# PJLab-ADG/OpenPCSeg

Measured on AMD Instinct MI355X. Metric: LiDAR frames/sec training MinkUNet-34 SemanticKITTI, higher is better.
Workload: dtype f32; 1 GPU; MinkUNet-34 cr1.0 train step, 12 x 120k-pt synthetic SemanticKITTI scans/GPU, fp32; global_batch=12, voxels_per_gpu_batch=1158864, parallelism=dp1, wgrad=fp32

## Files before the change

### openpcseg_amd/csrc/conv_wgrad.hip

```cpp
#include "conv_common.h"

using namespace pcs;

namespace {

constexpr int WG_PB = 32;
constexpr int WG_TS = 128 + 16;

struct WgradArgs {
  const float *fa;
  const float *fb;
  const int32_t *pairs;
  const int32_t *koff;
  float *partial;
  int ca, cb, K, a_col, pch;
};

__device__ __forceinline__ void find_split(const int32_t *koff, int K, int pch, int split, int *k_out,
                                           int *beg, int *end) {
  int acc = 0;
  for (int k = 0; k < K; ++k) {
    const int nk = koff[k + 1] - koff[k];
    const int ns = (nk + pch - 1) / pch;
    if (split < acc + ns) {
      const int s = split - acc;
      *k_out = k;
      *beg = koff[k] + s * pch;
      const int e = *beg + pch;
      *end = e < koff[k + 1] ? e : koff[k + 1];
      return;
    }
    acc += ns;
  }
  *k_out = -1; *beg = 0; *end = 0;
}

__device__ __forceinline__ void find_split_wave(const int32_t *koff, int K, int pch, int split, int lane, int *beg,
                                                int *end, int *gsid, int interleave) {
  if (K > 64) {
    int k;
    find_split(koff, K, pch, split, &k, beg, end);
    *gsid = split;
    return;
  }
  const int lo = lane < K ? koff[lane] : 0, hi = lane < K ? koff[lane + 1] : 0;
  const int ns = (hi - lo + pch - 1) / pch;
  int incl = ns;
  for (int o = 1; o < 64; o <<= 1) {
    const int t = __shfl_up(incl, o, 64);
    if (lane >= o) incl += t;
  }
  int src, sidx;
  if (!interleave) {
    const unsigned long long hit = __ballot(split >= incl - ns && split < incl);
    if (!hit) { *beg = 0; *end = 0; *gsid = split; return; }
    src = __ffsll((long long)hit) - 1;
    sidx = split - __shfl(incl - ns, src, 64);
  } else {
    const int total = __shfl(incl, 63, 64);
    if (interleave == 2) {
      const int chunk = (total + 7) >> 3;
      split = (split & 7) * chunk + (split >> 3);
    }
    if (split >= total) { *beg = 0; *end = 0; *gsid = 0; return; }
    int rmax = ns;
    for (int o = 32; o > 0; o >>= 1) { const int t = __shfl_xor(rmax, o, 64); rmax = t > rmax ? t : rmax; }
    auto upto = [&](int r) {
      int c = ns > 0 ? (int)(((long long)r * ns) / rmax) + 1 : 0;
      for (int o = 32; o > 0; o >>= 1) c += __shfl_xor(c, o, 64);
      return c;
    };
    int a = 0, b = rmax - 1;
    while (a < b) {
      const int m = (a + b) >> 1;
      if (upto(m) > split) b = m; else a = m + 1;
    }
    const int r = a;
    const int before = r > 0 ? upto(r - 1) : 0;
    const int s_r = ns > 0 ? (int)(((long long)r * ns) / rmax) : -1;
    const int s_p = (ns > 0 && r > 0) ? (int)(((long long)(r - 1) * ns) / rmax) : -1;
    unsigned long long fresh = __ballot(ns > 0 && s_r != s_p);
    int want = split - before;
    while (want > 0) { fresh &= fresh - 1; --want; }
    src = __ffsll((long long)fresh) - 1;
    sidx = __shfl(s_r, src, 64);
  }
  const int b0 = lo + sidx * pch;
  const int e0 = b0 + pch < hi ? b0 + pch : hi;
  *beg = __shfl(b0, src, 64);
  *end = __shfl(e0, src, 64);
  *gsid = __shfl(incl - ns, src, 64) + sidx;
}

template <bool VEC>
__global__ void __launch_bounds__(256) wgrad_kernel(WgradArgs w) {
  __shared__ __attribute__((aligned(16))) float abuf[WG_PB * WG_TS];
  __shared__ __attribute__((aligned(16))) float bbuf[WG_PB * WG_TS];
  __shared__ int ia[WG_PB], ib[WG_PB];
  __shared__ int sh[3];
  const int tid = threadIdx.x, lane = tid & 63, wid = tid >> 6;
  const int a0 = blockIdx.y * 128, b0 = blockIdx.z * 128;
  const int cat = (w.ca - a0) < 128 ? (w.ca - a0) : 128;
  const int cbt = (w.cb - b0) < 128 ? (w.cb - b0) : 128;
  const int ta_n = (cat + 15) / 16, tb_n = (cbt + 15) / 16;
  if (tid == 0) find_split(w.koff, w.K, w.pch, blockIdx.x, &sh[0], &sh[1], &sh[2]);
  __syncthreads();
  const int beg = sh[1], end = sh[2];
  const int wa = wid >> 1, wb = wid & 1;
  f32x4 acc[4][4];
#pragma unroll
  for (int i = 0; i < 4; ++i)
#pragma unroll
    for (int j = 0; j < 4; ++j) acc[i][j] = (f32x4){0, 0, 0, 0};

  const int capad = ta_n * 16, cbpad = tb_n * 16;
  for (int p0 = beg; p0 < end; p0 += WG_PB) {
    const int np = (end - p0) < WG_PB ? (end - p0) : WG_PB;
    __syncthreads();
    if (tid < WG_PB) {
      int2 p = make_int2(-1, -1);
      if (tid < np) p = reinterpret_cast<const int2 *>(w.pairs)[p0 + tid];
      ia[tid] = w.a_col ? p.y : p.x;
      ib[tid] = w.a_col ? p.x : p.y;
    }
    __syncthreads();
    if (VEC) {
      for (int e = tid; e < WG_PB * (capad / 4); e += 256) {
        const int r = e / (capad / 4), c4 = (e % (capad / 4)) * 4;
        float4 v = make_float4(0.f, 0.f, 0.f, 0.f);
        if (r < np && c4 < cat) v = *reinterpret_cast<const float4 *>(w.fa + (int64_t)ia[r] * w.ca + a0 + c4);
        *reinterpret_cast<float4 *>(abuf + r * WG_TS + c4) = v;
      }
      for (int e = tid; e < WG_PB * (cbpad / 4); e += 256) {
        const int r = e / (cbpad / 4), c4 = (e % (cbpad / 4)) * 4;
        float4 v = make_float4(0.f, 0.f, 0.f, 0.f);
        if (r < np && c4 < cbt) v = *reinterpret_cast<const float4 *>(w.fb + (int64_t)ib[r] * w.cb + b0 + c4);
        *reinterpret_cast<float4 *>(bbuf + r * WG_TS + c4) = v;
      }
    } else {
      for (int e = tid; e < WG_PB * capad; e += 256) {
        const int r = e / capad, c = e % capad;
        abuf[r * WG_TS + c] = (r < np && c < cat) ? w.fa[(int64_t)ia[r] * w.ca + a0 + c] : 0.f;
      }
      for (int e = tid; e < WG_PB * cbpad; e += 256) {
        const int r = e / cbpad, c = e % cbpad;
        bbuf[r * WG_TS + c] = (r < np && c < cbt) ? w.fb[(int64_t)ib[r] * w.cb + b0 + c] : 0.f;
      }
    }
    __syncthreads();
    const int g = lane >> 4, l15 = lane & 15;
#pragma unroll
    for (int kk = 0; kk < WG_PB / 4; ++kk) {
      float av[4], bv[4];
#pragma unroll
      for (int i = 0; i < 4; ++i) {
        const int ta = wa + 2 * i;
        av[i] = (ta < ta_n) ? abuf[(kk * 4 + g) * WG_TS + ta * 16 + l15] : 0.f;
      }
#pragma unroll
      for (int j = 0; j < 4; ++j) {
        const int tb = wb + 2 * j;
        bv[j] = (tb < tb_n) ? bbuf[(kk * 4 + g) * WG_TS + tb * 16 + l15] : 0.f;
      }
#pragma unroll
      for (int i = 0; i < 4; ++i) {
        if (wa + 2 * i < ta_n) {
#pragma unroll
          for (int j = 0; j < 4; ++j) {
            if (wb + 2 * j < tb_n)
              acc[i][j] = __builtin_amdgcn_mfma_f32_16x16x4f32(av[i], bv[j], acc[i][j], 0, 0, 0);
          }
        }
      }
    }
  }
  float *out = w.partial + (int64_t)blockIdx.x * w.ca * w.cb;
  const int g = lane >> 4, l15 = lane & 15;
#pragma unroll
  for (int i = 0; i < 4; ++i) {
    const int ta = wa + 2 * i;
    if (ta >= ta_n) continue;
#pragma unroll
    for (int j = 0; j < 4; ++j) {
      const int tb = wb + 2 * j;
      if (tb >= tb_n) continue;
#pragma unroll
      for (int r = 0; r < 4; ++r) {
        const int ra = ta * 16 + g * 4 + r, cbv = tb * 16 + l15;
        if (ra < cat && cbv < cbt) out[(int64_t)(a0 + ra) * w.cb + b0 + cbv] = acc[i][j][r];
      }
    }
  }
}

__global__ void __launch_bounds__(256) wgrad_reduce_kernel(const float *__restrict__ partial,
                                                           const int32_t *__restrict__ koff,
                                                           int K, int pch, int64_t cc,
                                                           float *__restrict__ gW) {
  const int k = blockIdx.y;
  __shared__ int sh[2];
  if (threadIdx.x == 0) {
    int acc = 0;
    for (int q = 0; q < k; ++q) acc += (koff[q + 1] - koff[q] + pch - 1) / pch;
    sh[0] = acc;
    sh[1] = (koff[k + 1] - koff[k] + pch - 1) / pch;
  }
  __syncthreads();
  const int base = sh[0], ns = sh[1];
  for (int64_t e = (int64_t)blockIdx.x * blockDim.x + threadIdx.x; e < cc;
       e += (int64_t)gridDim.x * blockDim.x) {
    float s = 0.f;
    for (int q = 0; q < ns; ++q) s += partial[(int64_t)(base + q) * cc + e];
    gW[(int64_t)k * cc + e] = s;
  }
}

__global__ void __launch_bounds__(256) wgrad_reduce4_kernel(const float *__restrict__ partial,
                                                            const int32_t *__restrict__ koff,
                                                            int K, int pch, int64_t cc,
                                                            float *__restrict__ gW) {
  const int k = blockIdx.y;
  __shared__ int sh[2];
  __shared__ float4 red[16][16];
  if (threadIdx.x < 64) {
    const int lane = threadIdx.x;
    int acc = 0, mine = 0;
    if (K <= 64) {
      const int nsq = lane < K ? (koff[lane + 1] - koff[lane] + pch - 1) / pch : 0;
      int incl = nsq;
      for (int o = 1; o < 64; o <<= 1) {
        const int t = __shfl_up(incl, o, 64);
        if (lane >= o) incl += t;
      }
      acc = __shfl(incl - nsq, k, 64);
      mine = __shfl(nsq, k, 64);
    } else {
      for (int q = 0; q < k; ++q) acc += (koff[q + 1] - koff[q] + pch - 1) / pch;
      mine = (koff[k + 1] - koff[k] + pch - 1) / pch;
    }
    if (lane == 0) { sh[0] = acc; sh[1] = mine; }
  }
  __syncthreads();
  const int base = sh[0], ns = sh[1];
  const int et = threadIdx.x & 15, ql = threadIdx.x >> 4;
  const int64_t e = ((int64_t)blockIdx.x * 16 + et) * 4;
  const bool ok = e < cc;
  const float *p = partial + (int64_t)base * cc + (ok ? e : 0);
  float4 s0 = {0, 0, 0, 0}, s1 = s0, s2 = s0, s3 = s0;
  int q = ql;
  for (; q + 48 < ns; q += 64) {
    const float4 v0 = *reinterpret_cast<const float4 *>(p + (int64_t)q * cc);
    const float4 v1 = *reinterpret_cast<const float4 *>(p + (int64_t)(q + 16) * cc);
    const float4 v2 = *reinterpret_cast<const float4 *>(p + (int64_t)(q + 32) * cc);
    const float4 v3 = *reinterpret_cast<const float4 *>(p + (int64_t)(q + 48) * cc);
    s0.x += v0.x; s0.y += v0.y; s0.z += v0.z; s0.w += v0.w;
    s1.x += v1.x; s1.y += v1.y; s1.z += v1.z; s1.w += v1.w;
    s2.x += v2.x; s2.y += v2.y; s2.z += v2.z; s2.w += v2.w;
    s3.x += v3.x; s3.y += v3.y; s3.z += v3.z; s3.w += v3.w;
  }
  for (; q < ns; q += 16) {
    const float4 v0 = *reinterpret_cast<const float4 *>(p + (int64_t)q * cc);
    s0.x += v0.x; s0.y += v0.y; s0.z += v0.z; s0.w += v0.w;
  }
  s0.x += s1.x + (s2.x + s3.x); s0.y += s1.y + (s2.y + s3.y);
  s0.z += s1.z + (s2.z + s3.z); s0.w += s1.w + (s2.w + s3.w);
  red[ql][et] = s0;
  __syncthreads();
  if (ql == 0 && ok) {
    float4 t = red[0][et];
#pragma unroll
    for (int j = 1; j < 16; ++j) {
      const float4 v = red[j][et];
      t.x += v.x; t.y += v.y; t.z += v.z; t.w += v.w;
    }
    *reinterpret_cast<float4 *>(gW + (int64_t)k * cc + e) = t;
  }
}

struct Wgrad2Args {
  const void *fa;
  const void *fb;
  const int32_t *pairs;
  const int32_t *koff;
  float *partial;
  int ca, cb, K, a_col, pch, nbg;
  int interleave;
};

__host__ __device__ inline int wg_ngroups(int c) { return (c + 63) / 64; }
__host__ __device__ inline int wg_gwidth(int c) {
  const int per = (c + wg_ngroups(c) - 1) / wg_ngroups(c);
  return (per + 15) / 16 * 16;
}

template <int W> struct WVec;
template <> struct WVec<64> { using T = float4; static constexpr int N = 4; };
template <> struct WVec<48> { using T = float3; static constexpr int N = 3; };
template <> struct WVec<32> { using T = float2; static constexpr int N = 2; };
template <> struct WVec<16> { using T = float;  static constexpr int N = 1; };
__device__ __forceinline__ float wcomp(const float4 &v, int i) { return i == 0 ? v.x : (i == 1 ? v.y : (i == 2 ? v.z : v.w)); }
__device__ __forceinline__ float wcomp(const float3 &v, int i) { return i == 0 ? v.x : (i == 1 ? v.y : v.z); }
__device__ __forceinline__ float wcomp(const float2 &v, int i) { return i == 0 ? v.x : v.y; }
__device__ __forceinline__ float wcomp(const float &v, int) { return v; }

template <typename V, int N> __device__ __forceinline__ V wload(Fp32, const void *base, int64_t elem) {
  return *reinterpret_cast<const V *>(reinterpret_cast<const float *>(base) + elem);
}
template <typename V, int N, typename HT> __device__ __forceinline__ V wload(HT, const void *base, int64_t elem) {
  const uint16_t *p = reinterpret_cast<const uint16_t *>(base) + elem;
  V v;
  if constexpr (N == 4) {
    const uint2 r = *reinterpret_cast<const uint2 *>(p);
    v.x = h2f(HT{}, (uint16_t)(r.x & 0xFFFFu)); v.y = h2f(HT{}, (uint16_t)(r.x >> 16));
    v.z = h2f(HT{}, (uint16_t)(r.y & 0xFFFFu)); v.w = h2f(HT{}, (uint16_t)(r.y >> 16));
  } else if constexpr (N == 3) {
    v.x = h2f(HT{}, p[0]); v.y = h2f(HT{}, p[1]); v.z = h2f(HT{}, p[2]);
  } else if constexpr (N == 2) {
    const uint32_t r = *reinterpret_cast<const uint32_t *>(p);
    v.x = h2f(HT{}, (uint16_t)(r & 0xFFFFu)); v.y = h2f(HT{}, (uint16_t)(r >> 16));
  } else {
    v = h2f(HT{}, p[0]);
  }
  return v;
}

template <int AW, int BW, typename ET>
__device__ __forceinline__ void wgrad_block(const Wgrad2Args &w, int a0, int b0, int beg, int end,
                                            float *out, int lane) {
  using AV = typename WVec<AW>::T;
  using BV = typename WVec<BW>::T;
  constexpr int NA = WVec<AW>::N, NB = WVec<BW>::N;
  const int g = lane >> 4, l15 = lane & 15;
  const int ac = a0 + NA * l15, bc = b0 + NB * l15;
  const bool aok = ac + NA <= w.ca, bok = bc + NB <= w.cb;
  const int acl = aok ? ac : 0, bcl = bok ? bc : 0;
  f32x4 acc[NA][NB];
#pragma unroll
  for (int f = 0; f < NA; ++f)
#pragma unroll
    for (int h = 0; h < NB; ++h) acc[f][h] = (f32x4){0, 0, 0, 0};

  struct Batch { AV a[4]; BV b[4]; };
  auto load_pairs = [&](int p0) {
    int pi = p0 + l15;
    pi = pi < end ? pi : end - 1;
    return reinterpret_cast<const int2 *>(w.pairs)[pi];
  };
  auto load_rows = [&](Batch &bt, const int2 pr) {
    const int ia = w.a_col ? pr.y : pr.x, ib = w.a_col ? pr.x : pr.y;
#pragma unroll
    for (int j = 0; j < 4; ++j) {
      const int ra = __shfl(ia, 4 * j + g, 64), rb = __shfl(ib, 4 * j + g, 64);
      bt.a[j] = wload<AV, NA>(ET{}, w.fa, (int64_t)ra * w.ca + acl);
      bt.b[j] = wload<BV, NB>(ET{}, w.fb, (int64_t)rb * w.cb + bcl);
    }
  };
  auto mfma_batch = [&](const Batch &bt, int p0) {
#pragma unroll
    for (int j = 0; j < 4; ++j) {
      const bool pv = aok && (p0 + 4 * j + g) < end;
#pragma unroll
      for (int f = 0; f < NA; ++f) {
        const float av = pv ? wcomp(bt.a[j], f) : 0.f;
#pragma unroll
        for (int h = 0; h < NB; ++h)
          acc[f][h] = __builtin_amdgcn_mfma_f32_16x16x4f32(av, wcomp(bt.b[j], h), acc[f][h], 0, 0, 0);
      }
    }
  };
  Batch b0s, b1s;
  load_rows(b0s, load_pairs(beg));
  int2 prn = load_pairs(beg + 16 < end ? beg + 16 : beg);
#ifndef PCS_ABLATEW
#define PCS_ABLATEW 0
#endif
#if PCS_ABLATEW == 1
  load_rows(b1s, prn);
#endif
  for (int p0 = beg; p0 < end; p0 += 32) {
    const int p2 = p0 + 32 < end ? p0 + 32 : p0;
    const int p3 = p0 + 48 < end ? p0 + 48 : p0;
#if PCS_ABLATEW != 1
    load_rows(b1s, prn);
#endif
    prn = load_pairs(p2);
    __builtin_amdgcn_sched_barrier(0);
#if PCS_ABLATEW != 2
    mfma_batch(b0s, p0);
#else
    acc[0][0][0] += wcomp(b0s.a[0], 0) + wcomp(b0s.a[1], 0) + wcomp(b0s.a[2], 0) + wcomp(b0s.a[3], 0) + wcomp(b0s.b[0], 0) + wcomp(b0s.b[1], 0) + wcomp(b0s.b[2], 0) + wcomp(b0s.b[3], 0);
#endif
    __builtin_amdgcn_sched_barrier(0);
#if PCS_ABLATEW != 1
    load_rows(b0s, prn);
#endif
    prn = load_pairs(p3);
    __builtin_amdgcn_sched_barrier(0);
#if PCS_ABLATEW != 2
    if (p0 + 16 < end) mfma_batch(b1s, p0 + 16);
#else
    acc[0][0][1] += wcomp(b1s.a[0], 0) + wcomp(b1s.a[1], 0) + wcomp(b1s.a[2], 0) + wcomp(b1s.a[3], 0) + wcomp(b1s.b[0], 0) + wcomp(b1s.b[1], 0) + wcomp(b1s.b[2], 0) + wcomp(b1s.b[3], 0);
#endif
    __builtin_amdgcn_sched_barrier(0);
  }
#pragma unroll
  for (int f = 0; f < NA; ++f) {
#pragma unroll
    for (int r = 0; r < 4; ++r) {
      const int row = a0 + NA * (4 * g + r) + f;
      if (row < w.ca && bok) {
        float *d = out + (int64_t)row * w.cb + bc;
#pragma unroll
        for (int h = 0; h < NB; ++h) d[h] = acc[f][h][r];
      }
    }
  }
}

template <typename ET>
__global__ void __launch_bounds__(256, 3) wgrad2_kernel(Wgrad2Args w) {
  const int tid = threadIdx.x, lane = tid & 63, wid = tid >> 6;
  int beg, end, gsid;
  find_split_wave(w.koff, w.K, w.pch, blockIdx.x, lane, &beg, &end, &gsid, w.interleave);
  const int nag = wg_ngroups(w.ca);
  const int nsb = (w.nbg + 1) >> 1;
  const int sa = blockIdx.y / nsb, sb = blockIdx.y - sa * nsb;
  const int ag = 2 * sa + (wid >> 1), bg = 2 * sb + (wid & 1);
  if (beg >= end || ag >= nag || bg >= w.nbg) return;
  const int aw = wg_gwidth(w.ca), bw = wg_gwidth(w.cb);
  float *out = w.partial + (int64_t)gsid * w.ca * w.cb;
  const int a0 = aw * ag, b0 = bw * bg;
#define PCS_WG_CASE(A, B) if (aw == A && bw == B) { wgrad_block<A, B, ET>(w, a0, b0, beg, end, out, lane); return; }
  PCS_WG_CASE(64, 64) PCS_WG_CASE(64, 48) PCS_WG_CASE(64, 32) PCS_WG_CASE(64, 16)
  PCS_WG_CASE(48, 64) PCS_WG_CASE(48, 48) PCS_WG_CASE(48, 32) PCS_WG_CASE(48, 16)
  PCS_WG_CASE(32, 64) PCS_WG_CASE(32, 48) PCS_WG_CASE(32, 32) PCS_WG_CASE(32, 16)
  PCS_WG_CASE(16, 64) PCS_WG_CASE(16, 48) PCS_WG_CASE(16, 32) PCS_WG_CASE(16, 16)
#undef PCS_WG_CASE
}

constexpr int W3_PB = 32;
constexpr int W3_ROW = 128;

typedef __bf16 w3_bf16x2 __attribute__((ext_vector_type(2)));
typedef float w3_f32x2 __attribute__((ext_vector_type(2)));
typedef __bf16 w3_bf16x8 __attribute__((ext_vector_type(8)));
typedef _Float16 w3_f16x8 __attribute__((ext_vector_type(8)));

struct Wgrad3Args {
  const void *fa;
  const void *fb;
  const int32_t *pairs;
  const int32_t *koff;
  float *partial;
  int ca, cb, K, a_col, pch;
  int aw, bw, nag, nbg, nsb;
  int interleave;
  int nsy = 1;
};

template <typename ET> struct W3Mode;
template <> struct W3Mode<Fp32> { static constexpr int PLANES = 3; using MT = Bf16; };
template <> struct W3Mode<Bf16> { static constexpr int PLANES = 1; using MT = Bf16; };
template <> struct W3Mode<Fp16> { static constexpr int PLANES = 1; using MT = Fp16; };

__device__ __forceinline__ f32x4 w3_mfma(Bf16, const uint4 &a, const uint4 &b, f32x4 c) {
  return __builtin_amdgcn_mfma_f32_16x16x32_bf16(__builtin_bit_cast(w3_bf16x8, a), __builtin_bit_cast(w3_bf16x8, b), c, 0, 0, 0);
}
__device__ __forceinline__ f32x4 w3_mfma(Fp16, const uint4 &a, const uint4 &b, f32x4 c) {
  return __builtin_amdgcn_mfma_f32_16x16x32_f16(__builtin_bit_cast(w3_f16x8, a), __builtin_bit_cast(w3_f16x8, b), c, 0, 0, 0);
}

__device__ __forceinline__ void w3_split(float x, float y, uint32_t &hi, uint32_t &mid, uint32_t &lo) {
  const w3_f32x2 v = {x, y};
  const w3_bf16x2 h = __builtin_convertvector(v, w3_bf16x2);
  const w3_f32x2 r1 = v - __builtin_convertvector(h, w3_f32x2);
  const w3_bf16x2 m = __builtin_convertvector(r1, w3_bf16x2);
  const w3_f32x2 r2 = r1 - __builtin_convertvector(m, w3_f32x2);
  const w3_bf16x2 l = __builtin_convertvector(r2, w3_bf16x2);
  hi = __builtin_bit_cast(uint32_t, h); mid = __builtin_bit_cast(uint32_t, m); lo = __builtin_bit_cast(uint32_t, l);
}

template <typename ET, int NA, int NB, int NT = 256, int ROW = W3_ROW>
__global__ void __launch_bounds__(NT, NT == 256 ? (W3Mode<ET>::PLANES == 1 ? 3 : 2) : 4) wgrad3_kernel(Wgrad3Args w) {
  constexpr int PL = W3Mode<ET>::PLANES;
  using MT = typename W3Mode<ET>::MT;
  constexpr bool F32IN = std::is_same<ET, Fp32>::value;
  constexpr int NBUF = PL == 1 ? 2 : 1;
  constexpr int IMG = PL * 2 * W3_PB * ROW;
  __shared__ __attribute__((aligned(16))) uint16_t lds[NBUF * IMG];
  const int tid = threadIdx.x, lane = tid & 63, wid = tid >> 6;
  const int g = lane >> 4, l15 = lane & 15;
  int beg, end, gsid;
  int bx = blockIdx.x, by = blockIdx.y;
  if (w.interleave == 2 && w.nsy > 1) {
    const int slot = bx >> 3;
    by = slot % w.nsy;
    bx = ((slot / w.nsy) << 3) | (bx & 7);
  }
  find_split_wave(w.koff, w.K, w.pch, bx, lane, &beg, &end, &gsid, w.interleave);
  if (beg >= end) return;
  const int sa = by / w.nsb, sb = by - sa * w.nsb;
  const int a_base = 2 * sa * w.aw, b_base = 2 * sb * w.bw;
  const int a_stage = (w.ca - a_base) < 2 * w.aw ? (w.ca - a_base) : 2 * w.aw;
  const int b_stage = (w.cb - b_base) < 2 * w.bw ? (w.cb - b_base) : 2 * w.bw;
  const int ag = 2 * sa + (wid >> 1), bg = 2 * sb + (wid & 1);
  const bool active = ag < w.nag && bg < w.nbg;
  const int aoff = (wid >> 1) * w.aw, boff = (wid & 1) * w.bw;

  f32x4 acc[NA][NB];
#pragma unroll
  for (int i = 0; i < NA; ++i)
#pragma unroll
    for (int j = 0; j < NB; ++j) acc[i][j] = (f32x4){0, 0, 0, 0};

  constexpr int CPP = F32IN ? 4 : 8;
  constexpr int PPR = ROW / CPP;
  constexpr int PIECES = (W3_PB / 2) * PPR / NT;
  static_assert(PIECES >= 1 && (W3_PB / 2) * PPR % NT == 0, "staging items must divide over the threads");
  uint32_t *ldw = reinterpret_cast<uint32_t *>(lds);
  constexpr int IMGW = IMG / 2;
  constexpr int OPW = (W3_PB / 2) * ROW;
  auto wpos = [](int q, int ch) { return q * ROW + ((((ch >> 4) ^ (q >> 2)) & (ROW / 16 - 1)) << 4) + (ch & 15); };
  int2 prs[PIECES][2];
  uint4 ra[PIECES][2], rb[PIECES][2];
  auto fetch_pairs = [&](int p0) {
#pragma unroll
    for (int i = 0; i < PIECES; ++i) {
      const int q = (tid + NT * i) / PPR;
#pragma unroll
      for (int h = 0; h < 2; ++h) {
        prs[i][h] = make_int2(-1, -1);
        if (p0 + 2 * q + h < end) prs[i][h] = reinterpret_cast<const int2 *>(w.pairs)[p0 + 2 * q + h];
      }
    }
  };
  auto fetch_rows = [&]() {
#pragma unroll
    for (int i = 0; i < PIECES; ++i) {
      const int c = ((tid + NT * i) % PPR) * CPP;
#pragma unroll
      for (int h = 0; h < 2; ++h) {
        const bool pv = prs[i][h].x >= 0;
        const int ia = w.a_col ? prs[i][h].y : prs[i][h].x, ib = w.a_col ? prs[i][h].x : prs[i][h].y;
        ra[i][h] = make_uint4(0u, 0u, 0u, 0u);
        rb[i][h] = make_uint4(0u, 0u, 0u, 0u);
        if (pv && c < a_stage) {
          if (F32IN) ra[i][h] = *reinterpret_cast<const uint4 *>(reinterpret_cast<const float *>(w.fa) + (int64_t)ia * w.ca + a_base + c);
          else ra[i][h] = *reinterpret_cast<const uint4 *>(reinterpret_cast<const uint16_t *>(w.fa) + (int64_t)ia * w.ca + a_base + c);
        }
        if (pv && c < b_stage) {
          if (F32IN) rb[i][h] = *reinterpret_cast<const uint4 *>(reinterpret_cast<const float *>(w.fb) + (int64_t)ib * w.cb + b_base + c);
          else rb[i][h] = *reinterpret_cast<const uint4 *>(reinterpret_cast<const uint16_t *>(w.fb) + (int64_t)ib * w.cb + b_base + c);
        }
      }
    }
  };
  auto stage = [&](int buf) {
#pragma unroll
    for (int i = 0; i < PIECES; ++i) {
      const int e = tid + NT * i, q = e / PPR, c = (e % PPR) * CPP;
      const int pos = wpos(q, c);
#pragma unroll
      for (int op = 0; op < 2; ++op) {
        const uint4 v0 = op ? rb[i][0] : ra[i][0], v1 = op ? rb[i][1] : ra[i][1];
        uint32_t *base = ldw + buf * IMGW + op * OPW + pos;
        if (F32IN) {
          uint4 hi, mid, lo;
          w3_split(__uint_as_float(v0.x), __uint_as_float(v1.x), hi.x, mid.x, lo.x);
          w3_split(__uint_as_float(v0.y), __uint_as_float(v1.y), hi.y, mid.y, lo.y);
          w3_split(__uint_as_float(v0.z), __uint_as_float(v1.z), hi.z, mid.z, lo.z);
          w3_split(__uint_as_float(v0.w), __uint_as_float(v1.w), hi.w, mid.w, lo.w);
          *reinterpret_cast<uint4 *>(base) = hi;
          *reinterpret_cast<uint4 *>(base + 2 * OPW) = mid;
          *reinterpret_cast<uint4 *>(base + 4 * OPW) = lo;
        } else {
          uint4 w0, w1;
          w0.x = __builtin_amdgcn_perm(v1.x, v0.x, 0x05040100u); w0.y = __builtin_amdgcn_perm(v1.x, v0.x, 0x07060302u);
          w0.z = __builtin_amdgcn_perm(v1.y, v0.y, 0x05040100u); w0.w = __builtin_amdgcn_perm(v1.y, v0.y, 0x07060302u);
          w1.x = __builtin_amdgcn_perm(v1.z, v0.z, 0x05040100u); w1.y = __builtin_amdgcn_perm(v1.z, v0.z, 0x07060302u);
          w1.z = __builtin_amdgcn_perm(v1.w, v0.w, 0x05040100u); w1.w = __builtin_amdgcn_perm(v1.w, v0.w, 0x07060302u);
          *reinterpret_cast<uint4 *>(base) = w0;
          *reinterpret_cast<uint4 *>(base + 4) = w1;
// ... 29 lines not shown
        for (int j = 0; j < NB; ++j) acc[i][j] = w3_mfma(MT{}, af[PL / 2], bf[j][0], acc[i][j]);
#pragma unroll
        for (int j = 0; j < NB; ++j) acc[i][j] = w3_mfma(MT{}, af[0], bf[j][PL / 2], acc[i][j]);
      }
#pragma unroll
      for (int j = 0; j < NB; ++j) acc[i][j] = w3_mfma(MT{}, af[0], bf[j][0], acc[i][j]);
    }
  };

  fetch_pairs(beg);
  fetch_rows();
  fetch_pairs(beg + W3_PB);
  stage(0);
  __syncthreads();
  int cur = 0;
  for (int p0 = beg; p0 < end; p0 += W3_PB) {
    const bool more = p0 + W3_PB < end;
    if (more) {
      fetch_rows();
      fetch_pairs(p0 + 2 * W3_PB);
    }
    if (active) compute(cur);
    if (NBUF == 2) {
      if (more) stage(cur ^ 1);
      __syncthreads();
      cur ^= 1;
    } else {
      __syncthreads();
      if (more) stage(0);
      __syncthreads();
    }
  }
  if (!active) return;
  const int a0 = a_base + aoff, b0 = b_base + boff;
  float *out = w.partial + (int64_t)gsid * w.ca * w.cb;
#pragma unroll
  for (int i = 0; i < NA; ++i)
#pragma unroll
    for (int r = 0; r < 4; ++r) {
      const int row = a0 + 16 * i + 4 * g + r;
      if (row < w.ca) {
#pragma unroll
        for (int j = 0; j < NB; ++j) {
          const int col = b0 + 16 * j + l15;
          if (col < w.cb) out[(int64_t)row * w.cb + col] = acc[i][j][r];
        }
      }
    }
}

template <typename ET>
int launch_wgrad3(const Wgrad3Args &w, int ns, hipStream_t st) {
  const int nsa = (w.nag + 1) / 2;
  const int nsy = nsa * w.nsb;
  const dim3 grid = w.interleave == 2 ? dim3((unsigned)(8 * ((ns + 7) / 8) * nsy), 1u) : dim3((unsigned)ns, (unsigned)nsy);
  const int na = w.aw / 16, nb = w.bw / 16;
#define PCS_W3_CASE(A, B) if (na == A && nb == B) { hipLaunchKernelGGL((wgrad3_kernel<ET, A, B>), grid, dim3(256), 0, st, w); return check_launch("pcs_conv_wgrad(wgrad3)"); }
  PCS_W3_CASE(4, 4) PCS_W3_CASE(4, 3) PCS_W3_CASE(4, 2) PCS_W3_CASE(4, 1)
  PCS_W3_CASE(3, 4) PCS_W3_CASE(3, 3) PCS_W3_CASE(3, 2) PCS_W3_CASE(3, 1)
  PCS_W3_CASE(2, 4) PCS_W3_CASE(2, 3) PCS_W3_CASE(2, 2) PCS_W3_CASE(2, 1)
  PCS_W3_CASE(1, 4) PCS_W3_CASE(1, 3) PCS_W3_CASE(1, 2) PCS_W3_CASE(1, 1)
#undef PCS_W3_CASE
  set_error("pcs_conv_wgrad(wgrad3): unreachable");
  return PCS_EINVAL;
}

inline bool wgrad3_thin(int ca, int cb, int dtype) {
  static const int on = getenv("PCS_WGRAD3_THIN") ? atoi(getenv("PCS_WGRAD3_THIN")) : 1;
  return on && dtype != 0 && ca % 16 == 0 && cb % 16 == 0 && ca <= 64 && cb <= 64 && ca >= 32 && cb >= 32;
}

template <typename ET>
int launch_wgrad3_thin(const Wgrad3Args &w, int ns, hipStream_t st) {
  const dim3 grid((unsigned)(w.interleave == 2 ? 8 * ((ns + 7) / 8) : ns), 1);
  const int na = w.aw / 16, nb = w.bw / 16;
#define PCS_W3T_CASE(A, B) if (na == A && nb == B) { hipLaunchKernelGGL((wgrad3_kernel<ET, A, B, 64, 64>), grid, dim3(64), 0, st, w); return check_launch("pcs_conv_wgrad(wgrad3 thin)"); }
  PCS_W3T_CASE(4, 4) PCS_W3T_CASE(4, 3) PCS_W3T_CASE(4, 2) PCS_W3T_CASE(3, 4) PCS_W3T_CASE(3, 3) PCS_W3T_CASE(3, 2)
  PCS_W3T_CASE(2, 4) PCS_W3T_CASE(2, 3) PCS_W3T_CASE(2, 2)
#undef PCS_W3T_CASE
  set_error("pcs_conv_wgrad(wgrad3 thin): unreachable");
  return PCS_EINVAL;
}

int wgrad_plan(const int32_t *koff_host, int K, int ca, int cb, int *pch_out, bool thin = false, bool half = false) {
  const int nbq = (wg_ngroups(ca) * wg_ngroups(cb) + 3) / 4;
  int64_t P = koff_host[K] - koff_host[0];
  static const int tgt_env = getenv("PCS_WGRAD_TARGET") ? atoi(getenv("PCS_WGRAD_TARGET")) : 0;
  int64_t target = (tgt_env > 0 ? tgt_env : (nbq >= 4 ? (half ? 2048 : 3072) : 1536)) / nbq;
  if (thin) target *= 4;
  if (target < K) target = K;
  int pch = (int)ceil_div(P > 0 ? P : 1, target);
  pch = (int)(ceil_div(pch, 32) * 32);
  if (pch < 64) pch = 64;
  int64_t ns = 0;
  for (int k = 0; k < K; ++k) ns += ceil_div((int64_t)koff_host[k + 1] - koff_host[k], pch);
  *pch_out = pch;
  return (int)ns;
}

}

extern "C" size_t pcs_conv_wgrad_ws_bytes(const int32_t *koff_host, int32_t K, int32_t ca,
                                          int32_t cb) {
  if (!koff_host || K <= 0 || ca <= 0 || cb <= 0) return 0;
  int pch;
  int ns = wgrad_plan(koff_host, K, ca, cb, &pch);
  if (wgrad3_thin(ca, cb, 1)) {
    const int ns_thin = wgrad_plan(koff_host, K, ca, cb, &pch, true);
    ns = ns_thin > ns ? ns_thin : ns;
  }
  const int ns_half = wgrad_plan(koff_host, K, ca, cb, &pch, false, true);
  ns = ns_half > ns ? ns_half : ns;
  return (size_t)(ns > 0 ? ns : 1) * ca * cb * sizeof(float);
}

static int g_wgrad_interleave = -1;
extern "C" void pcs_debug_wgrad_interleave(int32_t mode) { g_wgrad_interleave = mode; }

static int conv_wgrad_any(const void *fa_v, int32_t ca, const void *fb_v, int32_t cb,
                          const int32_t *pairs, int32_t a_col, const int32_t *koff_dev,
                          const int32_t *koff_host, int32_t K, float *gW, void *ws,
                          size_t ws_bytes, int dtype, void *stream, bool force_split = false) {
  const float *fa = reinterpret_cast<const float *>(fa_v), *fb = reinterpret_cast<const float *>(fb_v);
  if (ca <= 0 || cb <= 0 || K <= 0 || !koff_dev || !koff_host || !gW || (a_col != 0 && a_col != 1) || dtype < 0 || dtype > 2) {
    set_error("pcs_conv_wgrad_f32: bad args");
    return PCS_EINVAL;
  }
  hipStream_t st = as_stream(stream);
  int pch;
  static const int use3_thin = getenv("PCS_WGRAD3") ? atoi(getenv("PCS_WGRAD3")) : 1;
  const bool thin = use3_thin >= 1 && wgrad3_thin(ca, cb, dtype) && (((uintptr_t)fa_v | (uintptr_t)fb_v) & 15) == 0;
  const int ns = wgrad_plan(koff_host, K, ca, cb, &pch, thin, dtype != 0);
  const int64_t cc = (int64_t)ca * cb;
  if (ns == 0) {
    if (hipMemsetAsync(gW, 0, (size_t)K * cc * 4, st) != hipSuccess) { set_error("pcs_conv_wgrad_f32: memset failed"); return PCS_ELAUNCH; }
    return PCS_OK;
  }
  if (!fa || !fb || !pairs || !ws) { set_error("pcs_conv_wgrad_f32: null pointer"); return PCS_EINVAL; }
  if (ws_bytes < (size_t)ns * cc * 4) { set_error("pcs_conv_wgrad_f32: workspace too small"); return PCS_EWORKSPACE; }
  WgradArgs w;
  w.fa = fa; w.fb = fb; w.pairs = pairs; w.koff = koff_dev; w.partial = reinterpret_cast<float *>(ws);
  w.ca = ca; w.cb = cb; w.K = K; w.a_col = a_col; w.pch = pch;
  const bool vec = (ca % 4 == 0) && (cb % 4 == 0) && (((uintptr_t)fa | (uintptr_t)fb) & 15) == 0;
  if (dtype != 0 && !vec) { set_error("pcs_conv_wgrad_h: half operands need channel counts that are multiples of 4 and 16-byte aligned tensors"); return PCS_EUNSUPPORTED; }
  static const int use3 = getenv("PCS_WGRAD3") ? atoi(getenv("PCS_WGRAD3")) : 1;
  static const int interleave_env = getenv("PCS_WGRAD_INTERLEAVE") ? atoi(getenv("PCS_WGRAD_INTERLEAVE")) : -1;
  const int interleave = g_wgrad_interleave >= 0 ? g_wgrad_interleave : (interleave_env >= 0 ? interleave_env : (dtype != 0 ? 2 : 0));
  const int cgran = dtype == 0 ? 4 : 8;
  const bool want3 = dtype == 0 ? (use3 == 2 || force_split) : (use3 >= 1 && (use3 == 2 || wg_ngroups(ca) * wg_ngroups(cb) >= 4));
  if (thin) {
    Wgrad3Args w3;
    w3.fa = fa_v; w3.fb = fb_v; w3.pairs = pairs; w3.koff = koff_dev; w3.partial = reinterpret_cast<float *>(ws);
    w3.ca = ca; w3.cb = cb; w3.K = K; w3.a_col = a_col; w3.pch = pch;
    w3.aw = wg_gwidth(ca); w3.bw = wg_gwidth(cb); w3.nag = 1; w3.nbg = 1; w3.nsb = 1; w3.interleave = interleave;
    int rc3 = dtype == 1 ? launch_wgrad3_thin<Bf16>(w3, ns, st) : launch_wgrad3_thin<Fp16>(w3, ns, st);
    if (rc3) return rc3;
  } else if (vec && want3 && ca % cgran == 0 && cb % cgran == 0) {
    Wgrad3Args w3;
    w3.fa = fa_v; w3.fb = fb_v; w3.pairs = pairs; w3.koff = koff_dev; w3.partial = reinterpret_cast<float *>(ws);
    w3.ca = ca; w3.cb = cb; w3.K = K; w3.a_col = a_col; w3.pch = pch;
    w3.aw = wg_gwidth(ca); w3.bw = wg_gwidth(cb); w3.nag = wg_ngroups(ca); w3.nbg = wg_ngroups(cb); w3.nsb = (w3.nbg + 1) / 2;
    w3.interleave = interleave;
    w3.nsy = ((w3.nag + 1) / 2) * w3.nsb;
    int rc3 = dtype == 0 ? launch_wgrad3<Fp32>(w3, ns, st) : (dtype == 1 ? launch_wgrad3<Bf16>(w3, ns, st) : launch_wgrad3<Fp16>(w3, ns, st));
    if (rc3) return rc3;
  } else if (vec) {
    Wgrad2Args w2;
    w2.fa = fa; w2.fb = fb; w2.pairs = pairs; w2.koff = koff_dev; w2.partial = reinterpret_cast<float *>(ws);
    w2.ca = ca; w2.cb = cb; w2.K = K; w2.a_col = a_col; w2.pch = pch; w2.nbg = wg_ngroups(cb); w2.interleave = interleave;
    const dim3 grid2((unsigned)(interleave == 2 ? 8 * ((ns + 7) / 8) : ns), (unsigned)(((wg_ngroups(ca) + 1) / 2) * ((wg_ngroups(cb) + 1) / 2)));
    if (dtype == 0) hipLaunchKernelGGL(wgrad2_kernel<Fp32>, grid2, dim3(256), 0, st, w2);
    else if (dtype == 1) hipLaunchKernelGGL(wgrad2_kernel<Bf16>, grid2, dim3(256), 0, st, w2);
    else hipLaunchKernelGGL(wgrad2_kernel<Fp16>, grid2, dim3(256), 0, st, w2);
  } else {
    dim3 grid((unsigned)ns, (unsigned)ceil_div(ca, 128), (unsigned)ceil_div(cb, 128));
    hipLaunchKernelGGL(wgrad_kernel<false>, grid, dim3(256), 0, st, w);
  }
  int rc = check_launch("pcs_conv_wgrad_f32");
  if (rc) return rc;
  if (vec && (((uintptr_t)ws | (uintptr_t)gW) & 15) == 0) {
    hipLaunchKernelGGL(wgrad_reduce4_kernel, dim3((unsigned)ceil_div(cc, 64), K), dim3(256), 0, st,
                       reinterpret_cast<const float *>(ws), koff_dev, (int)K, pch, cc, gW);
  } else {
    int gx = (int)ceil_div(cc, 256);
    if (gx > 64) gx = 64;
    hipLaunchKernelGGL(wgrad_reduce_kernel, dim3(gx, K), dim3(256), 0, st,
                       reinterpret_cast<const float *>(ws), koff_dev, (int)K, pch, cc, gW);
  }
  return check_launch("pcs_conv_wgrad_f32(reduce)");
}

extern "C" int pcs_conv_wgrad_f32(const float *fa, int32_t ca, const float *fb, int32_t cb,
                                  const int32_t *pairs, int32_t a_col, const int32_t *koff_dev,
                                  const int32_t *koff_host, int32_t K, float *gW, void *ws,
                                  size_t ws_bytes, void *stream) {
  return conv_wgrad_any(fa, ca, fb, cb, pairs, a_col, koff_dev, koff_host, K, gW, ws, ws_bytes, 0, stream);
}

extern "C" int pcs_conv_wgrad_h(const void *fa, int32_t ca, const void *fb, int32_t cb,
                                const int32_t *pairs, int32_t a_col, const int32_t *koff_dev,
                                const int32_t *koff_host, int32_t K, float *gW, void *ws,
                                size_t ws_bytes, int32_t dtype, void *stream) {
  if (dtype != 1 && dtype != 2) { set_error("pcs_conv_wgrad_h: dtype must be 1 (bf16) or 2 (fp16)"); return PCS_EINVAL; }
  return conv_wgrad_any(fa, ca, fb, cb, pairs, a_col, koff_dev, koff_host, K, gW, ws, ws_bytes, dtype, stream);
}

extern "C" int pcs_conv_wgrad_f32_bf16x3(const float *fa, int32_t ca, const float *fb, int32_t cb,
                                         const int32_t *pairs, int32_t a_col, const int32_t *koff_dev,
                                         const int32_t *koff_host, int32_t K, float *gW, void *ws,
                                         size_t ws_bytes, void *stream) {
  if ((ca % 4) || (cb % 4) || (((uintptr_t)fa | (uintptr_t)fb) & 15)) { set_error("pcs_conv_wgrad_f32_bf16x3: needs 16-byte granular rows"); return PCS_EUNSUPPORTED; }
  return conv_wgrad_any(fa, ca, fb, cb, pairs, a_col, koff_dev, koff_host, K, gW, ws, ws_bytes, 0, stream, true);
}
```

Measured before the change: 105.3 frames/s.

## Add thin-wave wgrad2 variants and finer tail chunks for fp32 weight gradients

The fp32 wgrad2 path gains 1- and 2-wave block variants for layers with only one 64-channel group on a side, plus shape-specialized template instances that avoid runtime width dispatch. It also adds a split plan in which the last pairs of the pair list are cut into smaller chunks, sized from the measured resident block count, and linearizes the grid so those tail blocks fill idle CUs at the end of the launch. The aim is better occupancy and less end-of-kernel load imbalance. In exchange it creates more partial slices, which adds reduce work and workspace, and it adds occupancy queries on the host plus optional trace instrumentation.

New measurement: 105.3 frames/s, median of 2. Within noise of the previous version (+0.0%).

```diff
diff --git a/openpcseg_amd/csrc/conv_wgrad.hip b/openpcseg_amd/csrc/conv_wgrad.hip
--- a/openpcseg_amd/csrc/conv_wgrad.hip
+++ b/openpcseg_amd/csrc/conv_wgrad.hip
@@ -6,6 +6,31 @@
 
 constexpr int WG_PB = 32;
 constexpr int WG_TS = 128 + 16;
+
+struct WPlan { int pch, cut, tch; };
+constexpr int kNoCut = 0x7fffffff;
+
+__host__ __device__ inline int wplan_mid(const WPlan &p, int lo, int hi) {
+  const int m = p.cut > lo ? p.cut : lo;
+  return m < hi ? m : hi;
+}
+__host__ __device__ inline int wplan_count(const WPlan &p, int lo, int hi) {
+  const int m = wplan_mid(p, lo, hi);
+  return (m - lo + p.pch - 1) / p.pch + (hi - m + p.tch - 1) / p.tch;
+}
+__host__ __device__ inline void wplan_range(const WPlan &p, int lo, int hi, int s, int *beg, int *end) {
+  const int m = wplan_mid(p, lo, hi);
+  const int nb = (m - lo + p.pch - 1) / p.pch;
+  if (s < nb) {
+    const int b = lo + s * p.pch;
+    *beg = b;
+    *end = b + p.pch < m ? b + p.pch : m;
+  } else {
+    const int b = m + (s - nb) * p.tch;
+    *beg = b;
+    *end = b + p.tch < hi ? b + p.tch : hi;
+  }
+}
 
 struct WgradArgs {
   const float *fa;
@@ -13,21 +38,19 @@
   const int32_t *pairs;
   const int32_t *koff;
   float *partial;
-  int ca, cb, K, a_col, pch;
+  int ca, cb, K, a_col;
+  WPlan plan;
 };
 
-__device__ __forceinline__ void find_split(const int32_t *koff, int K, int pch, int split, int *k_out,
+__device__ __forceinline__ void find_split(const int32_t *koff, int K, const WPlan &plan, int split, int *k_out,
                                            int *beg, int *end) {
   int acc = 0;
   for (int k = 0; k < K; ++k) {
-    const int nk = koff[k + 1] - koff[k];
-    const int ns = (nk + pch - 1) / pch;
+    const int lo = koff[k], hi = koff[k + 1];
+    const int ns = wplan_count(plan, lo, hi);
     if (split < acc + ns) {
-      const int s = split - acc;
       *k_out = k;
-      *beg = koff[k] + s * pch;
-      const int e = *beg + pch;
-      *end = e < koff[k + 1] ? e : koff[k + 1];
+      wplan_range(plan, lo, hi, split - acc, beg, end);
       return;
     }
     acc += ns;
@@ -35,16 +58,16 @@
   *k_out = -1; *beg = 0; *end = 0;
 }
 
-__device__ __forceinline__ void find_split_wave(const int32_t *koff, int K, int pch, int split, int lane, int *beg,
+__device__ __forceinline__ void find_split_wave(const int32_t *koff, int K, const WPlan &plan, int split, int lane, int *beg,
                                                 int *end, int *gsid, int interleave) {
   if (K > 64) {
     int k;
-    find_split(koff, K, pch, split, &k, beg, end);
+    find_split(koff, K, plan, split, &k, beg, end);
     *gsid = split;
     return;
   }
   const int lo = lane < K ? koff[lane] : 0, hi = lane < K ? koff[lane + 1] : 0;
-  const int ns = (hi - lo + pch - 1) / pch;
+  const int ns = wplan_count(plan, lo, hi);
   int incl = ns;
   for (int o = 1; o < 64; o <<= 1) {
     const int t = __shfl_up(incl, o, 64);
@@ -85,8 +108,8 @@
     src = __ffsll((long long)fresh) - 1;
     sidx = __shfl(s_r, src, 64);
   }
-  const int b0 = lo + sidx * pch;
-  const int e0 = b0 + pch < hi ? b0 + pch : hi;
+  int b0, e0;
+  wplan_range(plan, lo, hi, sidx, &b0, &e0);
   *beg = __shfl(b0, src, 64);
   *end = __shfl(e0, src, 64);
   *gsid = __shfl(incl - ns, src, 64) + sidx;
@@ -103,7 +126,7 @@
   const int cat = (w.ca - a0) < 128 ? (w.ca - a0) : 128;
   const int cbt = (w.cb - b0) < 128 ? (w.cb - b0) : 128;
   const int ta_n = (cat + 15) / 16, tb_n = (cbt + 15) / 16;
-  if (tid == 0) find_split(w.koff, w.K, w.pch, blockIdx.x, &sh[0], &sh[1], &sh[2]);
+  if (tid == 0) find_split(w.koff, w.K, w.plan, blockIdx.x, &sh[0], &sh[1], &sh[2]);
   __syncthreads();
   const int beg = sh[1], end = sh[2];
   const int wa = wid >> 1, wb = wid & 1;
@@ -195,15 +218,15 @@
 
 __global__ void __launch_bounds__(256) wgrad_reduce_kernel(const float *__restrict__ partial,
                                                            const int32_t *__restrict__ koff,
-                                                           int K, int pch, int64_t cc,
+                                                           int K, WPlan plan, int64_t cc,
                                                            float *__restrict__ gW) {
   const int k = blockIdx.y;
   __shared__ int sh[2];
   if (threadIdx.x == 0) {
     int acc = 0;
-    for (int q = 0; q < k; ++q) acc += (koff[q + 1] - koff[q] + pch - 1) / pch;
+    for (int q = 0; q < k; ++q) acc += wplan_count(plan, koff[q], koff[q + 1]);
     sh[0] = acc;
-    sh[1] = (koff[k + 1] - koff[k] + pch - 1) / pch;
+    sh[1] = wplan_count(plan, koff[k], koff[k + 1]);
   }
   __syncthreads();
   const int base = sh[0], ns = sh[1];
@@ -217,7 +240,7 @@
 
 __global__ void __launch_bounds__(256) wgrad_reduce4_kernel(const float *__restrict__ partial,
                                                             const int32_t *__restrict__ koff,
-                                                            int K, int pch, int64_t cc,
+                                                            int K, WPlan plan, int64_t cc,
                                                             float *__restrict__ gW) {
   const int k = blockIdx.y;
   __shared__ int sh[2];
@@ -226,7 +249,7 @@
     const int lane = threadIdx.x;
     int acc = 0, mine = 0;
     if (K <= 64) {
-      const int nsq = lane < K ? (koff[lane + 1] - koff[lane] + pch - 1) / pch : 0;
+      const int nsq = lane < K ? wplan_count(plan, koff[lane], koff[lane + 1]) : 0;
       int incl = nsq;
       for (int o = 1; o < 64; o <<= 1) {
         const int t = __shfl_up(incl, o, 64);
@@ -235,8 +258,8 @@
       acc = __shfl(incl - nsq, k, 64);
       mine = __shfl(nsq, k, 64);
     } else {
-      for (int q = 0; q < k; ++q) acc += (koff[q + 1] - koff[q] + pch - 1) / pch;
-      mine = (koff[k + 1] - koff[k] + pch - 1) / pch;
+      for (int q = 0; q < k; ++q) acc += wplan_count(plan, koff[q], koff[q + 1]);
+      mine = wplan_count(plan, koff[k], koff[k + 1]);
     }
     if (lane == 0) { sh[0] = acc; sh[1] = mine; }
   }
@@ -283,8 +306,10 @@
   const int32_t *pairs;
   const int32_t *koff;
   float *partial;
-  int ca, cb, K, a_col, pch, nbg;
+  int ca, cb, K, a_col, nbg;
+  WPlan plan;
   int interleave;
+  int nsy;
 };
 
 __host__ __device__ inline int wg_ngroups(int c) { return (c + 63) / 64; }
@@ -417,26 +442,64 @@
   }
 }
 
-template <typename ET>
-__global__ void __launch_bounds__(256, 3) wgrad2_kernel(Wgrad2Args w) {
+#if PCS_TRACE
+__device__ long long *g_wgrad_trace;
+constexpr int kWTraceWaves = 1 << 16;
+#endif
+
+template <typename ET, int NW, int AW, int BW>
+__global__ void __launch_bounds__(64 * NW, 3) wgrad2_kernel(Wgrad2Args w) {
   const int tid = threadIdx.x, lane = tid & 63, wid = tid >> 6;
+  PCS_T(const long long tr_entry = wall_clock64();)
+  int bx = blockIdx.x, by = blockIdx.y;
+  if (w.nsy > 0) { by = bx % w.nsy; bx = bx / w.nsy; }
   int beg, end, gsid;
-  find_split_wave(w.koff, w.K, w.pch, blockIdx.x, lane, &beg, &end, &gsid, w.interleave);
+  find_split_wave(w.koff, w.K, w.plan, bx, lane, &beg, &end, &gsid, w.interleave);
   const int nag = wg_ngroups(w.ca);
-  const int nsb = (w.nbg + 1) >> 1;
-  const int sa = blockIdx.y / nsb, sb = blockIdx.y - sa * nsb;
-  const int ag = 2 * sa + (wid >> 1), bg = 2 * sb + (wid & 1);
+  int ag, bg;
+  if constexpr (NW == 4) {
+    const int nsb = (w.nbg + 1) >> 1;
+    const int sa = by / nsb, sb = by - sa * nsb;
+    ag = 2 * sa + (wid >> 1); bg = 2 * sb + (wid & 1);
+  } else if constexpr (NW == 2) {
+    ag = w.nbg == 1 ? 2 * by + wid : 0; bg = w.nbg == 1 ? 0 : 2 * by + wid;
+  } else {
+    ag = by / w.nbg; bg = by - ag * w.nbg;
+  }
   if (beg >= end || ag >= nag || bg >= w.nbg) return;
   const int aw = wg_gwidth(w.ca), bw = wg_gwidth(w.cb);
   float *out = w.partial + (int64_t)gsid * w.ca * w.cb;
   const int a0 = aw * ag, b0 = bw * bg;
-#define PCS_WG_CASE(A, B) if (aw == A && bw == B) { wgrad_block<A, B, ET>(w, a0, b0, beg, end, out, lane); return; }
-  PCS_WG_CASE(64, 64) PCS_WG_CASE(64, 48) PCS_WG_CASE(64, 32) PCS_WG_CASE(64, 16)
-  PCS_WG_CASE(48, 64) PCS_WG_CASE(48, 48) PCS_WG_CASE(48, 32) PCS_WG_CASE(48, 16)
-  PCS_WG_CASE(32, 64) PCS_WG_CASE(32, 48) PCS_WG_CASE(32, 32) PCS_WG_CASE(32, 16)
-  PCS_WG_CASE(16, 64) PCS_WG_CASE(16, 48) PCS_WG_CASE(16, 32) PCS_WG_CASE(16, 16)
+  if constexpr (AW != 0) {
+    wgrad_block<AW, BW, ET>(w, a0, b0, beg, end, out, lane);
+  } else {
+#define PCS_WG_CASE(A, B) if (aw == A && bw == B) wgrad_block<A, B, ET>(w, a0, b0, beg, end, out, lane); else
+    PCS_WG_CASE(64, 64) PCS_WG_CASE(64, 48) PCS_WG_CASE(64, 32) PCS_WG_CASE(64, 16)
+    PCS_WG_CASE(48, 64) PCS_WG_CASE(48, 48) PCS_WG_CASE(48, 32) PCS_WG_CASE(48, 16)
+    PCS_WG_CASE(32, 64) PCS_WG_CASE(32, 48) PCS_WG_CASE(32, 32) PCS_WG_CASE(32, 16)
+    PCS_WG_CASE(16, 64) PCS_WG_CASE(16, 48) PCS_WG_CASE(16, 32) PCS_WG_CASE(16, 16)
+    {}
 #undef PCS_WG_CASE
-}
+  }
+#if PCS_TRACE
+  const int64_t tr_id = ((int64_t)blockIdx.y * gridDim.x + blockIdx.x) * NW + wid;
+  if (lane == 0 && g_wgrad_trace && tr_id < kWTraceWaves) {
+    g_wgrad_trace[2 * tr_id] = tr_entry;
+    g_wgrad_trace[2 * tr_id + 1] = wall_clock64();
+  }
+#endif
+}
+
+#if PCS_TRACE
+long long *g_wtrace_host_ptr = nullptr;
+void wgrad_trace_reset(hipStream_t st) {
+  if (!g_wtrace_host_ptr) {
+    if (hipMalloc(&g_wtrace_host_ptr, (size_t)kWTraceWaves * 2 * sizeof(long long)) != hipSuccess) { g_wtrace_host_ptr = nullptr; return; }
+    (void)hipMemcpyToSymbol(HIP_SYMBOL(g_wgrad_trace), &g_wtrace_host_ptr, sizeof(g_wtrace_host_ptr));
+  }
+  (void)hipMemsetAsync(g_wtrace_host_ptr, 0, (size_t)kWTraceWaves * 2 * sizeof(long long), st);
+}
+#endif
 
 constexpr int W3_PB = 32;
 constexpr int W3_ROW = 128;
@@ -497,7 +560,7 @@
     by = slot % w.nsy;
     bx = ((slot / w.nsy) << 3) | (bx & 7);
   }
-  find_split_wave(w.koff, w.K, w.pch, bx, lane, &beg, &end, &gsid, w.interleave);
+  find_split_wave(w.koff, w.K, WPlan{w.pch, kNoCut, w.pch}, bx, lane, &beg, &end, &gsid, w.interleave);
   if (beg >= end) return;
   const int sa = by / w.nsb, sb = by - sa * w.nsb;
   const int a_base = 2 * sa * w.aw, b_base = 2 * sb * w.bw;
@@ -693,19 +756,81 @@
   return PCS_EINVAL;
 }
 
-int wgrad_plan(const int32_t *koff_host, int K, int ca, int cb, int *pch_out, bool thin = false, bool half = false) {
+inline int wgrad2_waves(int ca, int cb) {
+  static const int on = getenv("PCS_WGRAD2_THIN") ? atoi(getenv("PCS_WGRAD2_THIN")) : 1;
+  const int nag = wg_ngroups(ca), nbg = wg_ngroups(cb);
+  if (!on || (ca % 4) || (cb % 4)) return 4;
+  if (nag * nbg == 1) return 1;
+  return (nag == 1 || nbg == 1) ? (on == 2 ? 1 : 2) : 4;
+}
+inline int wgrad2_nsy(int ca, int cb, int nw) {
+  const int nag = wg_ngroups(ca), nbg = wg_ngroups(cb);
+  return nw == 4 ? ((nag + 1) / 2) * ((nbg + 1) / 2) : (nw == 2 ? (nag * nbg + 1) / 2 : nag * nbg);
+}
+
+typedef void (*Wgrad2Fn)(Wgrad2Args);
+inline Wgrad2Fn wgrad2_f32_kernel(int nw, int aw, int bw) {
+  if (nw == 4) return wgrad2_kernel<Fp32, 4, 0, 0>;
+#define PCS_WT_CASE(A, B) if (aw == A && bw == B) return nw == 1 ? wgrad2_kernel<Fp32, 1, A, B> : wgrad2_kernel<Fp32, 2, A, B>;
+  PCS_WT_CASE(64, 64) PCS_WT_CASE(64, 48) PCS_WT_CASE(64, 32) PCS_WT_CASE(64, 16)
+  PCS_WT_CASE(48, 64) PCS_WT_CASE(48, 48) PCS_WT_CASE(48, 32) PCS_WT_CASE(48, 16)
+  PCS_WT_CASE(32, 64) PCS_WT_CASE(32, 48) PCS_WT_CASE(32, 32) PCS_WT_CASE(32, 16)
+  PCS_WT_CASE(16, 64) PCS_WT_CASE(16, 48) PCS_WT_CASE(16, 32) PCS_WT_CASE(16, 16)
+#undef PCS_WT_CASE
+  return nullptr;
+}
+
+int wgrad2_resident(int nw, int aw, int bw) {
+  static int cus = 0;
+  static int per_cu[3][4][4];
+  if (cus == 0) {
+    int dev = 0, n = 0;
+    cus = (hipGetDevice(&dev) == hipSuccess && hipDeviceGetAttribute(&n, hipDeviceAttributeMultiprocessorCount, dev) == hipSuccess && n > 0) ? n : -1;
+    if (cus < 0) (void)hipGetLastError();
+  }
+  int &slot = per_cu[nw == 4 ? 2 : nw - 1][nw == 4 ? 0 : aw / 16 - 1][nw == 4 ? 0 : bw / 16 - 1];
+  if (slot == 0) {
+    int nb = 0;
+    const Wgrad2Fn fn = wgrad2_f32_kernel(nw, aw, bw);
+    if (cus > 0 && fn && hipOccupancyMaxActiveBlocksPerMultiprocessor(&nb, reinterpret_cast<const void *>(fn), 64 * nw, 0) == hipSuccess && nb > 0) {
+      slot = nb;
+    } else {
+      (void)hipGetLastError();
+      slot = 12 / nw;
+    }
+  }
+  return (cus > 0 ? cus : 256) * slot;
+}
+
+int wgrad_plan(const int32_t *koff_host, int K, int ca, int cb, WPlan *plan, bool thin = false, bool half = false, int nw = 4,
+               bool tail = false) {
   const int nbq = (wg_ngroups(ca) * wg_ngroups(cb) + 3) / 4;
   int64_t P = koff_host[K] - koff_host[0];
   static const int tgt_env = getenv("PCS_WGRAD_TARGET") ? atoi(getenv("PCS_WGRAD_TARGET")) : 0;
   int64_t target = (tgt_env > 0 ? tgt_env : (nbq >= 4 ? (half ? 2048 : 3072) : 1536)) / nbq;
   if (thin) target *= 4;
+  target *= 4 / nw;
   if (target < K) target = K;
   int pch = (int)ceil_div(P > 0 ? P : 1, target);
   pch = (int)(ceil_div(pch, 32) * 32);
   if (pch < 64) pch = 64;
+  plan->pch = pch; plan->cut = kNoCut; plan->tch = pch;
+  static const int tail_div = getenv("PCS_WGRAD_TAIL") ? atoi(getenv("PCS_WGRAD_TAIL")) : 4;
+  if (tail && tail_div > 1 && K <= 64 && P > 0) {
+    int tch = (int)(ceil_div(ceil_div(pch, tail_div), 32) * 32);
+    if (tch < 64) tch = 64;
+    if (tch < pch) {
+      const int nsy = wgrad2_nsy(ca, cb, nw);
+      int64_t nt = wgrad2_resident(nw, wg_gwidth(ca), wg_gwidth(cb)) / nsy;
+      if (nt < 1) nt = 1;
+      int64_t T = nt * tch;
+      if (T > P / 2) T = P / 2;
+      plan->cut = (int)(koff_host[K] - T);
+      plan->tch = tch;
+    }
+  }
   int64_t ns = 0;
-  for (int k = 0; k < K; ++k) ns += ceil_div((int64_t)koff_host[k + 1] - koff_host[k], pch);
-  *pch_out = pch;
+  for (int k = 0; k < K; ++k) ns += wplan_count(*plan, koff_host[k], koff_host[k + 1]);
   return (int)ns;
 }
 
@@ -714,14 +839,16 @@
 extern "C" size_t pcs_conv_wgrad_ws_bytes(const int32_t *koff_host, int32_t K, int32_t ca,
                                           int32_t cb) {
   if (!koff_host || K <= 0 || ca <= 0 || cb <= 0) return 0;
-  int pch;
-  int ns = wgrad_plan(koff_host, K, ca, cb, &pch);
+  WPlan plan;
+  int ns = wgrad_plan(koff_host, K, ca, cb, &plan);
   if (wgrad3_thin(ca, cb, 1)) {
-    const int ns_thin = wgrad_plan(koff_host, K, ca, cb, &pch, true);
+    const int ns_thin = wgrad_plan(koff_host, K, ca, cb, &plan, true);
     ns = ns_thin > ns ? ns_thin : ns;
   }
-  const int ns_half = wgrad_plan(koff_host, K, ca, cb, &pch, false, true);
+  const int ns_half = wgrad_plan(koff_host, K, ca, cb, &plan, false, true);
   ns = ns_half > ns ? ns_half : ns;
+  const int ns_f32 = wgrad_plan(koff_host, K, ca, cb, &plan, false, false, wgrad2_waves(ca, cb), true);
+  ns = ns_f32 > ns ? ns_f32 : ns;
   return (size_t)(ns > 0 ? ns : 1) * ca * cb * sizeof(float);
 }
 
@@ -738,10 +865,15 @@
     return PCS_EINVAL;
   }
   hipStream_t st = as_stream(stream);
-  int pch;
+  WPlan plan;
   static const int use3_thin = getenv("PCS_WGRAD3") ? atoi(getenv("PCS_WGRAD3")) : 1;
+  static const int use3 = getenv("PCS_WGRAD3") ? atoi(getenv("PCS_WGRAD3")) : 1;
   const bool thin = use3_thin >= 1 && wgrad3_thin(ca, cb, dtype) && (((uintptr_t)fa_v | (uintptr_t)fb_v) & 15) == 0;
-  const int ns = wgrad_plan(koff_host, K, ca, cb, &pch, thin, dtype != 0);
+  const bool vec = (ca % 4 == 0) && (cb % 4 == 0) && (((uintptr_t)fa | (uintptr_t)fb) & 15) == 0;
+  const bool f32k = dtype == 0 && vec && !(use3 == 2 || force_split);
+  const int nw = f32k ? wgrad2_waves(ca, cb) : 4;
+  const int ns = wgrad_plan(koff_host, K, ca, cb, &plan, thin, dtype != 0, nw, f32k);
+  const int pch = plan.pch;
   const int64_t cc = (int64_t)ca * cb;
   if (ns == 0) {
     if (hipMemsetAsync(gW, 0, (size_t)K * cc * 4, st) != hipSuccess) { set_error("pcs_conv_wgrad_f32: memset failed"); return PCS_ELAUNCH; }
@@ -751,10 +883,8 @@
   if (ws_bytes < (size_t)ns * cc * 4) { set_error("pcs_conv_wgrad_f32: workspace too small"); return PCS_EWORKSPACE; }
   WgradArgs w;
   w.fa = fa; w.fb = fb; w.pairs = pairs; w.koff = koff_dev; w.partial = reinterpret_cast<float *>(ws);
-  w.ca = ca; w.cb = cb; w.K = K; w.a_col = a_col; w.pch = pch;
-  const bool vec = (ca % 4 == 0) && (cb % 4 == 0) && (((uintptr_t)fa | (uintptr_t)fb) & 15) == 0;
+  w.ca = ca; w.cb = cb; w.K = K; w.a_col = a_col; w.plan = plan;
   if (dtype != 0 && !vec) { set_error("pcs_conv_wgrad_h: half operands need channel counts that are multiples of 4 and 16-byte aligned tensors"); return PCS_EUNSUPPORTED; }
-  static const int use3 = getenv("PCS_WGRAD3") ? atoi(getenv("PCS_WGRAD3")) : 1;
   static const int interleave_env = getenv("PCS_WGRAD_INTERLEAVE") ? atoi(getenv("PCS_WGRAD_INTERLEAVE")) : -1;
   const int interleave = g_wgrad_interleave >= 0 ? g_wgrad_interleave : (interleave_env >= 0 ? interleave_env : (dtype != 0 ? 2 : 0));
   const int cgran = dtype == 0 ? 4 : 8;
@@ -778,11 +908,17 @@
   } else if (vec) {
     Wgrad2Args w2;
     w2.fa = fa; w2.fb = fb; w2.pairs = pairs; w2.koff = koff_dev; w2.partial = reinterpret_cast<float *>(ws);
-    w2.ca = ca; w2.cb = cb; w2.K = K; w2.a_col = a_col; w2.pch = pch; w2.nbg = wg_ngroups(cb); w2.interleave = interleave;
-    const dim3 grid2((unsigned)(interleave == 2 ? 8 * ((ns + 7) / 8) : ns), (unsigned)(((wg_ngroups(ca) + 1) / 2) * ((wg_ngroups(cb) + 1) / 2)));
-    if (dtype == 0) hipLaunchKernelGGL(wgrad2_kernel<Fp32>, grid2, dim3(256), 0, st, w2);
-    else if (dtype == 1) hipLaunchKernelGGL(wgrad2_kernel<Bf16>, grid2, dim3(256), 0, st, w2);
-    else hipLaunchKernelGGL(wgrad2_kernel<Fp16>, grid2, dim3(256), 0, st, w2);
+    w2.ca = ca; w2.cb = cb; w2.K = K; w2.a_col = a_col; w2.plan = plan; w2.nbg = wg_ngroups(cb); w2.interleave = interleave;
+    const unsigned npos = (unsigned)(interleave == 2 ? 8 * ((ns + 7) / 8) : ns), nsy = (unsigned)wgrad2_nsy(ca, cb, nw);
+    w2.nsy = plan.cut != kNoCut ? (int)nsy : 0;
+    const dim3 grid2 = w2.nsy ? dim3(npos * nsy, 1u) : dim3(npos, nsy);
+    PCS_T(wgrad_trace_reset(st);)
+    if (dtype == 0) {
+      const Wgrad2Fn fn = wgrad2_f32_kernel(nw, wg_gwidth(ca), wg_gwidth(cb));
+      if (!fn) { set_error("pcs_conv_wgrad_f32: no kernel instance for this shape"); return PCS_EINVAL; }
+      hipLaunchKernelGGL(fn, grid2, dim3(64 * nw), 0, st, w2);
+    } else if (dtype == 1) hipLaunchKernelGGL((wgrad2_kernel<Bf16, 4, 0, 0>), grid2, dim3(256), 0, st, w2);
+    else hipLaunchKernelGGL((wgrad2_kernel<Fp16, 4, 0, 0>), grid2, dim3(256), 0, st, w2);
   } else {
     dim3 grid((unsigned)ns, (unsigned)ceil_div(ca, 128), (unsigned)ceil_div(cb, 128));
     hipLaunchKernelGGL(wgrad_kernel<false>, grid, dim3(256), 0, st, w);
@@ -791,12 +927,12 @@
   if (rc) return rc;
   if (vec && (((uintptr_t)ws | (uintptr_t)gW) & 15) == 0) {
     hipLaunchKernelGGL(wgrad_reduce4_kernel, dim3((unsigned)ceil_div(cc, 64), K), dim3(256), 0, st,
-                       reinterpret_cast<const float *>(ws), koff_dev, (int)K, pch, cc, gW);
+                       reinterpret_cast<const float *>(ws), koff_dev, (int)K, plan, cc, gW);
   } else {
     int gx = (int)ceil_div(cc, 256);
     if (gx > 64) gx = 64;
     hipLaunchKernelGGL(wgrad_reduce_kernel, dim3(gx, K), dim3(256), 0, st,
-                       reinterpret_cast<const float *>(ws), koff_dev, (int)K, pch, cc, gW);
+                       reinterpret_cast<const float *>(ws), koff_dev, (int)K, plan, cc, gW);
   }
   return check_launch("pcs_conv_wgrad_f32(reduce)");
 }
@@ -823,3 +959,11 @@
   if ((ca % 4) || (cb % 4) || (((uintptr_t)fa | (uintptr_t)fb) & 15)) { set_error("pcs_conv_wgrad_f32_bf16x3: needs 16-byte granular rows"); return PCS_EUNSUPPORTED; }
   return conv_wgrad_any(fa, ca, fb, cb, pairs, a_col, koff_dev, koff_host, K, gW, ws, ws_bytes, 0, stream, true);
 }
+
+#if PCS_TRACE
+extern "C" int pcs_debug_wgrad_trace(long long *host_out) {
+  if (!g_wtrace_host_ptr || !host_out) return PCS_EINVAL;
+  if (hipDeviceSynchronize() != hipSuccess) return PCS_ELAUNCH;
+  return hipMemcpy(host_out, g_wtrace_host_ptr, (size_t)kWTraceWaves * 2 * sizeof(long long), hipMemcpyDeviceToHost) == hipSuccess ? PCS_OK : PCS_ELAUNCH;
+}
+#endif
```
